# tonandr/keras_unsupervised

Hardware: AMD Instinct MI355X
Metric: cd1_gibbs_steps_per_sec (higher is better)
Workload: dtype f32 (storage, accumulation, results); products as exact bf16 triples on the bf16 MFMA (x3), the 0/1 x 0/1 product of the positive statistics on the fp8 MFMA (exact); 1 GPU; rbm_784x1024_cd1_batch4096_fp32 (BASELINE.json configs[1]); n_vis=784, n_hid=1024, batch_per_gpu=4096, global_batch=4096, cd_k=1, update_mode=fused, lr=1e-3/4096, parallelism=dp1, compute=x3

## Files before the change

keras_unsupervised_amd/csrc/kurbm_api.hip:

```cpp
#include <hip/hip_runtime.h>

#include <cstdarg>
#include <cstdio>
#include <cstdlib>
#include <cstring>
#include <string>

#include "../../include/kurbm.h"
#include "kurbm_kernels.h"
#include "kurbm_comm.h"

using namespace kurbm;

enum { KN_LDPAD, KN_X3_F8POS, KN_X3_BYTES, KN_X3_STATS_TALL, KN_BF16_SPLIT, KN_X3_FULL, KN_X3_TALL, KN_X3_MFAST, KN_X3_STATS_MFAST,
       KN_UNFUSED_MIRROR, KN_X3_XCD2D, KN_REDUCE_TR, KN_DP_CHUNKS, KN_X3_STATS_BYTES, KN_MAP_SLOW, KN_X3_PAIR, KN_X3_SPLIT_STATS, KN_X3_ATR, KN_SMALL_LOCAL,
       KN_COUNT };
constexpr int KN_AUTO = -1;
static const struct { const char* env; int dflt; } KNOBS[KN_COUNT] = {
    {"KURBM_LDPAD", 0},
    {"KURBM_X3_F8POS", 1},
    {"KURBM_X3_BYTES", 1},
    {"KURBM_X3_STATS_TALL", 1},
    {"KURBM_BF16_SPLIT", KN_AUTO},
    {"KURBM_X3_FULL", 0},
    {"KURBM_X3_TALL", KN_AUTO},
    {"KURBM_X3_MFAST", 1},
    {"KURBM_X3_STATS_MFAST", 0},
    {"KURBM_UNFUSED_MIRROR", 0},
    {"KURBM_X3_XCD2D", 1},
    {"KURBM_REDUCE_TR", 0},
    {"KURBM_DP_CHUNKS", 0},
    {"KURBM_X3_STATS_BYTES", 1},
    {"KURBM_MAP_SLOW", 0},
    {"KURBM_X3_PAIR", 1},
    {"KURBM_X3_SPLIT_STATS", 1},
    {"KURBM_X3_ATR", 1},
    {"KURBM_SMALL_LOCAL", 1},
};

constexpr size_t STATUS_BYTES = 4096;
struct kurbm_ctx {
    int device;
    int ncu;
    int force_cfg[3];
    int force_split;
    int tile_major;
    int knob[KN_COUNT];
    int xcc_round_robin;
    unsigned xcc_map;
    unsigned* status;
};

// ... 1114 lines not shown
    const size_t mb = carve_mirror(ctx, nullptr, p->n_vis, p->n_hid, pieces).bytes;
    if (mb > mirror_bytes) return fail(KURBM_ERR_WORKSPACE, "mirror too small: need %zu bytes, got %zu", mb, mirror_bytes);
    const size_t wb = carve_bf16(ctx, nullptr, rows > 0 ? rows : 1, p->n_vis, p->n_hid, pieces, v_pieces).bytes;
    if (wb > workspace_bytes) return fail(KURBM_ERR_WORKSPACE, "workspace too small: need %zu bytes, got %zu", wb, workspace_bytes);
    return KURBM_OK;
}

static bool split_stats_on(const kurbm_ctx* ctx, int pieces, int v_pieces) {
    return pieces == 3 && v_pieces == 3 && ctx->knob[KN_X3_SPLIT_STATS] != 0 && ctx->knob[KN_X3_BYTES] != 0;
}

static bool atr_on(const kurbm_ctx* ctx, int pieces, int v_pieces, bool gauss) {
    return gauss && split_stats_on(ctx, pieces, v_pieces) && ctx->knob[KN_X3_ATR] != 0 && ctx->knob[KN_X3_PAIR] != 0 && ctx->knob[KN_LDPAD] == 0;
}

static int cd_step_any(kurbm_ctx* ctx, int pieces, int v_pieces, const kurbm_params* p, void* mirror, size_t mirror_bytes,
                       const float* v_batch, int rows, int ldv, const kurbm_cd_opts* o, int which, void* workspace,
                       size_t workspace_bytes, kurbm_stream_t stream, int only = -1, int m_lo = 0, int m_hi = -1,
                       const kurbm_momentum* mom = nullptr) {
#define KURBM_STAGE(n) (only < 0 || only == (n) || (only == 8 && (n) <= 3) || (only == 7 && ((n) == 4 || (n) == 5)))
    if (m_hi < 0) m_hi = p ? p->n_vis : 0;
    if (int e = check_cd_args(ctx, pieces, v_pieces, p, mirror, mirror_bytes, v_batch, rows, ldv, o, workspace, workspace_bytes, false)) return e;
    if (mom) {
        if (int e = check_mom(mom, o)) return e;
        if (only >= 0) return fail(KURBM_ERR_ARG, "momentum applies to whole steps only");
    }
    const bool v_binary = (v_pieces == (1 | KURBM_V_BINARY));
    if (v_binary) v_pieces = 1;
    hipStream_t st = static_cast<hipStream_t>(stream);
    const Mirror m = carve_mirror(ctx, mirror, p->n_vis, p->n_hid, pieces);
    WorkspaceB w = carve_bf16(ctx, workspace, rows, p->n_vis, p->n_hid, pieces, v_pieces);

    const bool gauss = (o->mode == KURBM_MODE_VISIBLE_GAUSSIAN);
    const int act_h = gauss ? ACT_RELU : ACT_SIGMOID;
    const int act_v = gauss ? ACT_LINEAR : ACT_SIGMOID;
    const int noise_v = gauss ? NOISE_GAUSSIAN : NOISE_BERNOULLI;
    const uint32_t base = o->chain * 64u;
    const bool need_w = (which & 1) || o->delta_out;
    const int vn_pieces = (pieces == 3 && gauss) ? 3 : 1;
    const bool f8pos = v_binary && pieces == 3 && ctx->knob[KN_X3_F8POS] != 0;
    const bool byt = ctx->knob[KN_X3_BYTES] != 0;
    const bool hbytes = byt, vbytes = byt && v_binary && pieces == 3, nbytes = byt && !gauss;
    const bool tbytes = f8pos && nbytes && ctx->knob[KN_X3_STATS_BYTES] != 0 && ctx->knob[KN_X3_STATS_TALL] != 0 && p->n_vis > 128;
    const bool split_stats = split_stats_on(ctx, pieces, v_pieces);
    const bool tbytes_n = tbytes || (split_stats && nbytes);
    const bool vneg_tr = atr_on(ctx, pieces, v_pieces, gauss);
    int e;

    const int gp_v = ceil_div(rows, 64);
    const float* part_v_pos = nullptr;
    if (o->v_planes) {
        if (!aligned16(o->v_planes)) return fail(KURBM_ERR_ARG, "v_planes is misaligned");
        const VPlanes vp = carve_vplanes(ctx, o->v_planes, rows, p->n_vis, v_pieces);
        w.vb = vp.vb; w.vbT = vp.vbT; part_v_pos = vp.part_v;
    } else if (KURBM_STAGE(0))
        HIP_TRY(launch_f32_to_bf16(v_batch, rows, p->n_vis, ldv, w.vb, w.Lv, w.Kb, w.vbT, w.Lb, p->n_vis, v_pieces, w.planeV,
                                   w.planeVT, w.part_v, w.ldv32, st, f8pos ? 1 : 0, vbytes ? 1 : 0));
    RngArgs r = make_rng(o->seed, o->row0, base + 0u, o->step);
    if (KURBM_STAGE(1)) {
        HalfOutB ho;
        ho.out = w.hb; ho.ldo = w.Lh; ho.out_bytes = hbytes; ho.outT = w.hbT; ho.ldoT = w.Lb; ho.outT_f8 = f8pos; ho.outT_b8 = split_stats;
        ho.colpart = w.part_h; ho.ld_colpart = w.ldh32; ho.colsign = 1.f;
        if ((e = half_step_b(ctx, LAYOUT_VH, p, m, w.vb, w.Lv, v_pieces, w.planeV, rows, act_h, NOISE_BERNOULLI, &r, ho, st, vbytes))) return e;
    }
    const uint16_t* h_cur = w.hb;
    if (o->v_chain && KURBM_STAGE(1)) {
        HIP_TRY(launch_f32_to_bf16(o->v_chain, rows, p->n_vis, ldv, w.cb, w.Lv, w.Kb, nullptr, 0, 0, v_pieces, w.planeV, 0, nullptr, 0, st,
                                   0, vbytes ? 1 : 0));
        r = make_rng(o->seed, o->row0, base + 32u, o->step);
        HalfOutB ho;
        ho.out = w.h2b; ho.ldo = w.Lh; ho.out_bytes = hbytes;
        if ((e = half_step_b(ctx, LAYOUT_VH, p, m, w.cb, w.Lv, v_pieces, w.planeV, rows, act_h, NOISE_BERNOULLI, &r, ho, st, vbytes))) return e;
        h_cur = w.h2b;
    }
    int gm_v = ceil_div(rows, 128), gm_h = gm_v;
    for (int t = 1; t <= o->k; ++t) {
        const bool last = (t == o->k);
        r = make_rng(o->seed, o->row0, base + 2u * t - 1u, o->step);
        if (KURBM_STAGE(2)) {
            HalfOutB ho;
            ho.out = w.v2b; ho.ldo = w.Lv; ho.out_pieces = vn_pieces; ho.out_plane = w.planeV; ho.out_bytes = nbytes;
            if (last) {
                if (vneg_tr) ho.out_rows_pad = w.Kb;
                if (!vneg_tr) { ho.outT = w.v2bT; ho.ldoT = w.Lb; ho.outT_pieces = vn_pieces; ho.outT_plane = w.planeVT; ho.outT_b8 = tbytes_n; }
                ho.out_f32 = o->v_chain; ho.ldo32 = ldv;
                ho.grid_m_out = &gm_v;
            }
            ho.colpart = last ? w.part_v + (size_t)gp_v * w.ldv32 : nullptr; ho.ld_colpart = w.ldv32;
            ho.colsign = -1.f;
            if ((e = half_step_b(ctx, LAYOUT_HV, p, m, h_cur, w.Lh, 1, 0, rows, act_v, noise_v, &r, ho, st, hbytes))) return e;
        }
        if (!last && KURBM_STAGE(2)) {
            r = make_rng(o->seed, o->row0, base + 2u * t, o->step);
            HalfOutB ho;
            ho.out = w.h2b; ho.ldo = w.Lh; ho.out_bytes = hbytes;
            if ((e = half_step_b(ctx, LAYOUT_VH, p, m, w.v2b, w.Lv, vn_pieces, w.planeV, rows, act_h, NOISE_BERNOULLI, &r, ho, st, nbytes))) return e;
            h_cur = w.h2b;
        }
    }
// ... 87 lines not shown
            g.pb_max = 3;
            g.nseg = pb_codes(ctx, 1, 3, 0u, &g.seg_codes, 0);
            g.m_fastest = ctx->knob[KN_X3_STATS_MFAST];
            g.nkt = q.nkt; g.inv_nkt = inv_of(g.nkt);
            g.kt_total = q.kt_total; g.kt_per_split = q.kt_per_split; g.nsplit = q.nsplit;
            g.xcd2d = ctx->knob[KN_X3_XCD2D]; g.map_force = ctx->knob[KN_MAP_SLOW];
            HIP_TRY(launch_gemm_pb(EPI_SLAB, g, st));
        }
    } else if (need_w && KURBM_STAGE(4)) {
        GemmArgsB g;
        memset(&g, 0, sizeof g);
        g.A0 = w.vbT + (size_t)m_lo * w.Lb; g.a_plane0 = w.planeVT; g.B0 = w.hbT;
        g.A1 = w.v2bT + (size_t)m_lo * w.Lb; g.a_plane1 = w.planeVT; g.B1 = w.hnT; g.b_plane1 = w.planeHT;
        g.lda = w.Lb; g.ldb = w.Lb;
        if (tbytes) { g.a_bytes = 1; g.lda = 2 * w.Lb; }
        g.M = Mr; g.N = p->n_hid; g.K = w.Kb;
        g.grid_m = pl.gm; g.grid_n = pl.gn;
        g.slab = w.slab; g.slab_stride = slab_stride; g.ld_slab = pl.ld_slab;
        g.nseg = pb_codes(ctx, v_pieces, 1, 0u, &g.seg_codes, 0);
        g.nseg = pb_codes(ctx, vn_pieces, pieces, 1u, &g.seg_codes, g.nseg);
        g.pb_max = pieces;
        g.seg_fastest = 1; g.inv_nseg = inv_of(g.nseg);
        if (f8pos) { g.f8pos = 1; g.inv_nseg = inv_of(2 * g.nseg - 1); }
        g.m_fastest = ctx->knob[KN_X3_STATS_MFAST];
        g.cfg = pl.cfg;
        g.nkt = pl.nkt; g.inv_nkt = inv_of(g.nkt);
        g.kt_total = pl.kt_total; g.kt_per_split = pl.kt_per_split; g.nsplit = pl.nsplit;
        g.xcd2d = ctx->knob[KN_X3_XCD2D]; g.map_force = ctx->knob[KN_MAP_SLOW];
        HIP_TRY(launch_gemm_pb(EPI_SLAB, g, st));
    }
// ... 308 lines not shown
    a.rows = rows; a.n_vis = p->n_vis; a.ldv = ldv; a.ldv1 = w.ldv32; a.ncol_tiles = ncol0; a.ncol_tiles1 = ncol1; a.ld_rowpart = ld_rp;
    HIP_TRY(launch_score(a, st));
    return KURBM_OK;
}

int kurbm_x3_dump_plane(kurbm_ctx* ctx, int which, int rows, int n_vis, int n_hid, int v_pieces, int mode, const void* workspace,
                        size_t workspace_bytes, float* out, int ld_out, kurbm_stream_t stream) {
    if (!ctx || !workspace || !out) return fail(KURBM_ERR_ARG, "null argument");
    const bool v_binary = (v_pieces == (1 | KURBM_V_BINARY));
    if (v_binary) v_pieces = 1;
    if (rows <= 0 || n_vis <= 0 || n_hid <= 0 || (v_pieces != 1 && v_pieces != 3)) return fail(KURBM_ERR_ARG, "bad shape / v_pieces");
    const WorkspaceB w = carve_bf16(ctx, const_cast<void*>(workspace), rows, n_vis, n_hid, 3, v_pieces);
    if (w.bytes > workspace_bytes) return fail(KURBM_ERR_WORKSPACE, "workspace too small");
    const bool gauss = (mode == KURBM_MODE_VISIBLE_GAUSSIAN), byt = ctx->knob[KN_X3_BYTES] != 0;
    const bool f8pos = v_binary && ctx->knob[KN_X3_F8POS] != 0;
    DumpArgs a;
    memset(&a, 0, sizeof a);
    a.out = out; a.rows = rows; a.ld_out = ld_out; a.pieces = 1; a.sign = 1.f;
    switch (which) {
        case KURBM_PLANE_H_POS:   a.src = w.hb;   a.units = n_hid; a.ld = w.Lh; a.fmt = byt ? 1 : 0; break;
        case KURBM_PLANE_H_POS_T: a.src = w.hbT;  a.units = n_hid; a.ld = w.Lb; a.fmt = f8pos ? 2 : 0; a.transposed = 1;
                                  if (split_stats_on(ctx, 3, v_pieces)) { a.fmt = 1; a.ld = 2 * w.Lb; }
                                  break;
        case KURBM_PLANE_V_NEG:   a.src = w.v2b;  a.units = n_vis; a.ld = w.Lv; a.fmt = (byt && !gauss) ? 1 : 0;
                                  a.pieces = gauss ? 3 : 1; a.plane = w.planeV; break;
        case KURBM_PLANE_V_NEG_T: a.src = w.v2bT; a.units = n_vis; a.ld = w.Lb; a.transposed = 1;
                                  a.pieces = gauss ? 3 : 1; a.plane = w.planeVT;
                                  if (atr_on(ctx, 3, v_pieces, gauss)) {
                                      a.src = w.v2b; a.ld = w.Lv; a.transposed = 0; a.plane = w.planeV;
                                  }
                                  if ((f8pos && byt && !gauss && ctx->knob[KN_X3_STATS_BYTES] != 0 && ctx->knob[KN_X3_STATS_TALL] != 0 && n_vis > 128) ||
                                      (split_stats_on(ctx, 3, v_pieces) && !gauss)) {
                                      a.fmt = 1; a.ld = 2 * w.Lb;
                                  }
                                  break;
        case KURBM_PLANE_H_NEG_T: a.src = w.hnT;  a.units = n_hid; a.ld = w.Lb; a.transposed = 1; a.pieces = 3; a.plane = w.planeHT;
                                  a.sign = -1.f; break;
        default: return fail(KURBM_ERR_ARG, "unknown plane %d", which);
    }
    if (ld_out < a.units) return fail(KURBM_ERR_ARG, "ld_out < units");
    HIP_TRY(launch_dump_plane(a, static_cast<hipStream_t>(stream)));
    return KURBM_OK;
}

static int cd_epoch_x3_any(kurbm_ctx* ctx, const kurbm_params* p, void* mirror, size_t mirror_bytes, const float* V,
                           int v_pieces, int n_rows, int ldv, int batch_size, const kurbm_cd_opts* opts, void* workspace,
                           size_t workspace_bytes, kurbm_stream_t stream, const kurbm_momentum* mom) {
    if (!ctx || !opts) return fail(KURBM_ERR_ARG, "null argument");
    if (n_rows < 0 || batch_size <= 0) return fail(KURBM_ERR_ARG, "bad row count / batch size");
// ... 93 lines not shown
        if (b > bound[nc] && b < p->n_vis) bound[++nc] = b;
    }
    bound[++nc] = p->n_vis;
    kurbm_cd_opts o = *opts;
    o.apply = 0;
    const bool apply_ranges = opts->apply && nc > 1 && (p->n_hid & 3) == 0;
    if (rows == 0) HIP_TRY(hipMemsetAsync(o.delta_out, 0, ntot * sizeof(float), st));
    else if (nc > 1)
        if (int e = cd_step_any(ctx, pieces, v_pieces, p, mirror, mirror_bytes, v_batch, rows, ldv, &o, 7, workspace, workspace_bytes, stream, 8))
            return e;
    int err = KURBM_OK;
    bool on_comm = false;
    auto range = [&](int c) -> int {
        if (rows > 0) {
            const int e = (nc == 1)
                ? cd_step_any(ctx, pieces, v_pieces, p, mirror, mirror_bytes, v_batch, rows, ldv, &o, 7, workspace, workspace_bytes, stream)
                : cd_step_any(ctx, pieces, v_pieces, p, mirror, mirror_bytes, v_batch, rows, ldv, &o, 7, workspace, workspace_bytes, stream, 7,
                              bound[c], bound[c + 1]);
            if (e) return e;
        }
        const size_t lo = (size_t)bound[c] * p->n_hid, hi = (c + 1 == nc) ? ntot : (size_t)bound[c + 1] * p->n_hid;
        if (nc == 1)
            return comm_allreduce_sum(comm, o.delta_out + lo, hi - lo, st);
        HIP_TRY(hipEventRecord(comm->ev_ready[c], st));
        HIP_TRY(hipStreamWaitEvent(comm->stream, comm->ev_ready[c], 0));
        on_comm = true;
        if (int e = comm_allreduce_sum(comm, o.delta_out + lo, hi - lo, comm->stream)) return e;
        if (apply_ranges)
            return apply_delta_rows(ctx, p, mirror, mirror_bytes, pieces, o.delta_out, o.lr, 7, bound[c], bound[c + 1], c + 1 == nc, comm->stream);
        return KURBM_OK;
    };
// ... 18 lines not shown
int kurbm_cd_step_x3_peer(kurbm_ctx* ctx, kurbm_peer* peer, const kurbm_params* p, void* mirror, size_t mirror_bytes,
                          const float* v_batch, int v_pieces, int rows, int ldv, const kurbm_cd_opts* opts, void* workspace,
                          size_t workspace_bytes, kurbm_stream_t stream) {
    if (!ctx || !peer || !opts) return fail(KURBM_ERR_ARG, "null argument");
    if (int e = check_params(p)) return e;
    if (int e = peer_geometry_ok(peer, ctx->device, p->n_vis, p->n_hid)) return e;
    if (!opts->apply) return fail(KURBM_ERR_ARG, "kurbm_cd_step_x3_peer applies the summed update in place: apply = 1");
    if (rows < 0) return fail(KURBM_ERR_ARG, "rows must be >= 0");
    if (int e = check_cd_args(ctx, 3, v_pieces, p, mirror, mirror_bytes, v_batch, rows, ldv, opts, workspace, workspace_bytes, true)) return e;
    hipStream_t st = static_cast<hipStream_t>(stream);
    const size_t nw = (size_t)p->n_vis * p->n_hid, ntot = nw + p->n_hid + p->n_vis;
    kurbm_cd_opts o = *opts;
    o.apply = 0;
    o.delta_out = peer_delta(peer);
    if (rows == 0) HIP_TRY(hipMemsetAsync(o.delta_out, 0, ntot * sizeof(float), st));
    else if (int e = cd_step_any(ctx, 3, v_pieces, p, mirror, mirror_bytes, v_batch, rows, ldv, &o, 7, workspace, workspace_bytes, stream)) return e;
    PeerSrc src;
    if (int e = peer_exchange_shot1(peer, ctx->status, st, &src)) return e;
    const Mirror m = carve_mirror(ctx, mirror, p->n_vis, p->n_hid, 3);
    ReduceArgs a;
    memset(&a, 0, sizeof a);
    a.slab = src.own_sum; a.slab_stride = 0; a.nslab = 1; a.ld_slab = p->n_hid;
    a.n_vis = p->n_vis; a.n_hid = p->n_hid; a.ldw = p->ldw; a.lr = o.lr;
    a.W = p->W;
    a.part_h = src.own_sum + nw; a.nrow_tiles_h = 1; a.ld_part_h = p->n_hid; a.b_h = p->b_h;
    a.part_v = src.own_sum + nw + p->n_hid; a.nrow_tiles_v = 1; a.ld_part_v = p->n_vis; a.b_v = p->b_v;
    a.Wb = m.Wb; a.ldWb = m.ldW; a.planeWb = m.planeW;
    a.Wtb = m.Wtb; a.ldWtb = m.ldWt; a.planeWtb = m.planeWt; a.pieces = 3;
    a.tile_rows = ctx->knob[KN_REDUCE_TR];
    HIP_TRY(launch_reduce_apply_split(a, st, &src));
    return KURBM_OK;
// ... 77 lines not shown
```

keras_unsupervised_amd/csrc/kurbm_kernels.h:

```cpp
#pragma once
#include <hip/hip_runtime.h>
#include <stdint.h>

namespace kurbm {

enum { ACT_SIGMOID = 0, ACT_RELU = 1, ACT_LINEAR = 2 };
enum { NOISE_NONE = 0, NOISE_BERNOULLI = 1, NOISE_GAUSSIAN = 2 };
enum { EPI_HALFSTEP = 0, EPI_SLAB = 1, EPI_SOFTPLUS = 2, EPI_AIS = 3 };
enum { LAYOUT_VH = 0, LAYOUT_HV = 1, LAYOUT_OUTER = 2 };
enum { CFG_128x128 = 0, CFG_128x112 = 1, CFG_112x128 = 2, CFG_128x64 = 3, CFG_64x128 = 4, CFG_64x64 = 5,
       CFG_64x112 = 6, CFG_112x64 = 7, CFG_COUNT = 8 };

struct RngArgs {
    uint32_t seed_lo, seed_hi;
    uint32_t stream_id, step;
    uint64_t row0;
};

struct GemmArgs {
    const float* A0;
    const float* B0;
    const float* A1;
    const float* B1;
    int lda, ldb;
// ... 230 lines not shown
    int outT_f8;
    int outT_neg;
    size_t outT_plane;
    float* out_f32;
    float* prob_f32;
    float* out_u;
    int ldo32;
    float* colpart;
    int ld_colpart;
    float colsign;
    float* slab;
    size_t slab_stride;
    int ld_slab;
    int slab_t;
    int a_tr;
    int pair_ok;
    int map_force;
    int xcd2d;
    float* rowpart;
    int ld_rowpart;
    int rp;
    unsigned long long* stamps;
};

struct DumpArgs {
    const void* src;
    float* out;
    int rows, units, ld, ld_out, fmt, transposed, pieces;
    size_t plane;
    float sign;
// ... 52 lines not shown
```

keras_unsupervised_amd/csrc/kurbm_x3.hip:

```cpp
#include <hip/hip_runtime.h>
#include <hip/hip_ext.h>
#include <stdint.h>
#include <stdlib.h>

#include <type_traits>

#include "kurbm_kernels.h"
#include "kurbm_device.h"

namespace kurbm {

typedef __bf16 bf16x8 __attribute__((ext_vector_type(8)));
typedef uint32_t u32x4 __attribute__((ext_vector_type(4)));
typedef uint32_t u32x2 __attribute__((ext_vector_type(2)));

#ifdef KURBM_STAMPS
#define KURBM_STAMP(var)                                                                        \
    do {                                                                                        \
        __builtin_amdgcn_sched_barrier(0);                                                      \
        asm volatile("s_memtime %0\n\ts_waitcnt lgkmcnt(0)" : "=s"(var)::"memory");             \
        __builtin_amdgcn_sched_barrier(0);                                                      \
    } while (0)
#else
#define KURBM_STAMP(var) do { } while (0)
// ... 125 lines not shown
        const int tmn = bid - z * tiles_mn;
        const int q2 = div_map(tmn, g.m_fastest ? g.grid_m : g.grid_n, g.map_inv_b, g.map_slow);
        bm = g.m_fastest ? tmn - q2 * g.grid_m : q2;
        bn = g.m_fastest ? q2 : tmn - q2 * g.grid_n;
    }
    const int m0 = bm * BM, n0 = bn * BN;
    KURBM_PSTAMP(4);

    const int t_begin = z * g.kt_per_split;
    int t_end = t_begin + g.kt_per_split;
    if (t_end > g.kt_total) t_end = g.kt_total;
    const int nt = (t_end > t_begin && !(EPI == EPI_HALFSTEP && n0 >= g.N)) ? t_end - t_begin : 0;

    constexpr bool ATR = BSP && EPI == EPI_SLAB;
    const bool a_tr = ATR && g.a_tr != 0;
    unsigned goffA[NA], goffB[NB1];
#pragma unroll
    for (int it = 0; it < NA; ++it) {
        const int q = it * NTS + stid, row = q / CPR, ch = q % CPR;
        const int x = (m0 + row < g.M) ? m0 + row : 0;
        goffA[it] = AB ? (unsigned)(x * g.lda + 16 * (ch ^ ((row >> 1) & 7))) : 2u * (unsigned)(x * g.lda + 8 * (ch ^ ((row >> 1) & 7)));
        if (a_tr) {
            const int rt = q >> 4, ct = q & 15;
            goffA[it] = 2u * (unsigned)(rt * g.lda + m0 + 8 * (ct ^ (((rt & 3) << 2) | ((rt >> 2) & 3))));
        }
    }
#pragma unroll
    for (int it = 0; it < NB1; ++it) {
        const int q = it * NTS + stid, row = q / CPR, ch = q % CPR;
        const int x = (n0 + row < g.N) ? n0 + row : 0;
// ... 96 lines not shown
                    }
#endif
                    return;
                }
            }
            const unsigned char* c = smem + (bsp ? buf * A_BYTES : buf * STAGE) + (wm * WM + l15) * ROWB + 16 * ((4 * ks + slot) ^ swz);
#pragma unroll
            for (int mi = 0; mi < TM; ++mi) f[mi] = *reinterpret_cast<const u32x4*>(c + mi * 16 * ROWB);
        }
    };
    auto frag_b = [&](int buf, int ks, int p, u32x4 (&f)[TN]) __attribute__((always_inline)) {
        const unsigned char* c = smem + (bsp ? BSP_BOFF + buf * B_BYTES : buf * STAGE + B_OFF) + p * B1_BYTES + (wn * WN + l15) * ROWB +
                                 16 * ((4 * ks + slot) ^ swz);
#pragma unroll
        for (int ni = 0; ni < TN; ++ni) f[ni] = *reinterpret_cast<const u32x4*>(c + ni * 16 * ROWB);
    };
    [[maybe_unused]] u32x4 fx[AB ? TM : 1];
    auto expand_a = [&](int ks) __attribute__((always_inline)) {
        if constexpr (AB) {
#pragma unroll
            for (int mi = 0; mi < TM; ++mi) {
                const uint32_t lo = ks ? fa[0][mi].z : fa[0][mi].x, hi = ks ? fa[0][mi].w : fa[0][mi].y;
                fx[mi] = u32x4{__builtin_amdgcn_perm(0u, lo, 0x010C000Cu), __builtin_amdgcn_perm(0u, lo, 0x030C020Cu),
                               __builtin_amdgcn_perm(0u, hi, 0x010C000Cu), __builtin_amdgcn_perm(0u, hi, 0x030C020Cu)};
            }
        }
    };
    auto mfmas = [&](const afrag (&a)[TM], const u32x4 (&b)[TN]) __attribute__((always_inline)) {
#pragma unroll
        for (int mi = 0; mi < TM; ++mi) {
// ... 238 lines not shown
                }
                for (; i < nt; ++i) {
                    if (i + 3 < nt) __builtin_amdgcn_s_waitcnt(vm(NPT));
                    else __builtin_amdgcn_s_waitcnt(VM0);
                    __builtin_amdgcn_s_barrier();
                }
                KURBM_LSTAMP_OUT();
            } else if constexpr (ABS) {
                static_assert(NA / 2 + 3 * NB1 == 10 && NA + NB1 == 10, "10 pieces per wave and tile");
                const int nu = nt / 3;
                TileRef rp = tile_of(t_begin), rn = tile_of(t_begin + 1);
                TileRef ra = rn;
                ra.oa = rn.oa >> 1;
                int bf = 0, bb = 1;
                auto nxt = [](int b, int by) constexpr { return (b + by) % 3; };
                dma_part(2, rp, 3, bf);
                dma_part(0, ra, 1, bb);
                dma_part(0, rn, 2);
                __builtin_amdgcn_s_waitcnt(vm(NA + 3 * NB1));
                __builtin_amdgcn_s_setprio(KURBM_PRIO_LOADER);
                __builtin_amdgcn_s_barrier();
                rn.ob += 128u;
                for (int u = 0; u < nu; ++u) {
                    const bool more = u + 1 < nu;
                    const int bf1 = nxt(bf, 2), bb1 = nxt(bb, 2);
                    KURBM_LSTAMP(0);
                    if (more) { rp.oa += 128u; rp.ob += 128u; dma_part(0, rp, 1, bf1, 0, NA / 2); }
                    dma_part(1, rn, 2);
                    rn.ob += 128u;
                    KURBM_LSTAMP(1);
                    if (more) __builtin_amdgcn_s_waitcnt(vm(10)); else __builtin_amdgcn_s_waitcnt(vm(3 * NB1));
                    KURBM_LSTAMP(2);
                    __builtin_amdgcn_s_barrier();
                    KURBM_LSTAMP(3);
                    if (more) {
                        ra.oa += 128u;
                        dma_part(0, ra, 1, bb1, 0, NA / 2);
                        dma_part(2, rp, 2);
                        dma_part(0, rp, 1, bf1, NA / 2, NA);
                        __builtin_amdgcn_s_waitcnt(vm(10));
                    } else {
                        __builtin_amdgcn_s_waitcnt(VM0);
                    }
                    __builtin_amdgcn_s_barrier();
                    if (more) {
                        dma_part(0, rn, 2);
                        rn.ob += 128u;
                        dma_part(0, ra, 1, bb1, NA / 2, NA);
                        __builtin_amdgcn_s_waitcnt(vm(10));
                    } else {
                        __builtin_amdgcn_s_waitcnt(VM0);
                    }
                    __builtin_amdgcn_s_barrier();
                    bf = bf1; bb = bb1;
                }
                KURBM_LSTAMP_OUT();
            } else if constexpr (AB) {
                TileRef ra = tile_of(t_begin);
                TileRef rb = ra;
                const uint32_t ob0 = ra.ob;
                ra.neg = false; ra.oa = 128u * (uint32_t)(t_begin >> 1);
                KURBM_PSTAMP(0);
                dma_part(0, ra, 3, 0);
// ... 146 lines not shown
            for (int ni = 0; ni < NI_LDS; ++ni)
#pragma unroll
                for (int mi = 0; mi < TM; ++mi) {
                    const uint64_t grow = g.rng.row0 + (uint64_t)(m0 + wm * WM + slot * 4 + mi * 16);
                    uint32_t w[4];
                    philox4x32_10((uint32_t)(n0 + wn * WN + l15 + ni * 16), (uint32_t)(grow >> 2), g.rng.stream_id, g.rng.step,
                                  g.rng.seed_lo, g.rng.seed_hi, w);
                    *reinterpret_cast<u32x4*>(smem + SMEM_BYTES + ((ni * TM + mi) * NT + tid) * 16) = u32x4{w[0], w[1], w[2], w[3]};
                }
        }
    }
    __builtin_amdgcn_s_setprio(KURBM_PRIO_MFMA);
    if (nt > 0) {
        __syncthreads();
        frag_a(0, 0, fa[0]);
        frag_b(ABS ? 2 : 0, 0, 0, fb[0]);
        if constexpr (!ABS) expand_a(0);
        KURBM_STAMP(ts[1]);
        int i = 0;
        if constexpr (ABS) {
            const uint32_t arow = (uint32_t)((wm * WM + l15) * ROWB);
            uint32_t of8 = 0u, oby = A_BYTES;
            auto rd_f8 = [&](uint32_t off, int ks, afrag (&f)[TM]) __attribute__((always_inline)) {
                const unsigned char* c = smem + (arow + 16 * ((4 * ks + slot) ^ swz) + off);
#pragma unroll
                for (int mi = 0; mi < TM; ++mi) f[mi] = *reinterpret_cast<const u32x4*>(c + mi * 16 * ROWB);
            };
            auto rd_by = [&](uint32_t off, int half, afrag (&f)[TM]) __attribute__((always_inline)) {
                const unsigned char* c = smem + (arow + 16 * ((4 * half + slot) ^ swz) + off);
#pragma unroll
                for (int mi = 0; mi < TM; ++mi) f[mi] = *reinterpret_cast<const u32x4*>(c + mi * 16 * ROWB);
// ... 5 lines not shown
#pragma unroll
                for (int mi = 0; mi < TM; ++mi) {
                    const uint32_t lo = ks ? fa[0][mi].z : fa[0][mi].x, hi = ks ? fa[0][mi].w : fa[0][mi].y;
                    fa[1][mi] = u32x4{__builtin_amdgcn_perm(0u, lo, 0x010C000Cu), __builtin_amdgcn_perm(0u, lo, 0x030C020Cu),
                                      __builtin_amdgcn_perm(0u, hi, 0x010C000Cu), __builtin_amdgcn_perm(0u, hi, 0x030C020Cu)};
                }
            };
            auto mf = [&](const u32x4 (&b)[TN]) __attribute__((always_inline)) {
#pragma unroll
                for (int mi = 0; mi < TM; ++mi)
#pragma unroll
                    for (int ni = 0; ni < TN; ++ni)
                        acc[mi][ni] = __builtin_amdgcn_mfma_f32_16x16x32_bf16(
                            __builtin_bit_cast(bf16x8, fa[1][mi]), __builtin_bit_cast(bf16x8, b[ni]), acc[mi][ni], 0, 0, 0);
            };
            auto f8t = [&]() __attribute__((always_inline)) {
                typedef int i32x8 __attribute__((ext_vector_type(8)));
                __builtin_amdgcn_sched_barrier(0);
                rd_f8(of8, 1, fa[1]);
                frag_b(2, 1, 0, fb[1]);
#pragma unroll
                for (int mi = 0; mi < TM; ++mi)
#pragma unroll
                    for (int ni = 0; ni < TN; ++ni) {
                        const i32x8 a = {(int)fa[0][mi].x, (int)fa[0][mi].y, (int)fa[0][mi].z, (int)fa[0][mi].w,
                                         (int)fa[1][mi].x, (int)fa[1][mi].y, (int)fa[1][mi].z, (int)fa[1][mi].w};
                        const i32x8 b = {(int)fb[0][ni].x, (int)fb[0][ni].y, (int)fb[0][ni].z, (int)fb[0][ni].w,
                                         (int)fb[1][ni].x, (int)fb[1][ni].y, (int)fb[1][ni].z, (int)fb[1][ni].w};
                        acc[mi][ni] = __builtin_amdgcn_mfma_scale_f32_16x16x128_f8f6f4(a, b, acc[mi][ni], 0, 0, 0, 0x80, 0, 0x7F);
                    }
                __builtin_amdgcn_sched_barrier(0);
                __syncthreads();
                __builtin_amdgcn_sched_barrier(0);
                rd_by(oby, 0, fa[0]);
                frag_b(0, 0, 0, fb[0]);
                __builtin_amdgcn_sched_barrier(0);
                expand0(0);
                __builtin_amdgcn_sched_barrier(0);
            };
            auto negt = [&](const int half, const uint32_t nf8) __attribute__((always_inline)) {
#pragma unroll
                for (int u = 0; u < 6; ++u) {
                    __builtin_amdgcn_sched_barrier(0);
                    if (u == 0) { frag_b(half, 0, 1, fb[1]); frag_b(half, 0, 2, fb[2]); }
                    if (u == 1) frag_b(half, 1, 0, fb[0]);
                    if (u == 2) frag_b(half, 1, 1, fb[1]);
                    if (u == 3) frag_b(half, 1, 2, fb[2]);
                    if (u == 5) {
                        __syncthreads();
                        __builtin_amdgcn_sched_barrier(0);
                        if (half == 0) { rd_by(oby, 1, fa[0]); frag_b(1, 0, 0, fb[0]); }
                        else { rd_f8(nf8, 0, fa[0]); frag_b(2, 0, 0, fb[0]); }
                    }
                    mf(fb[u % 3]);
                    if (u == 2) { __builtin_amdgcn_sched_barrier(0); expand0(1); }
                    if (u == 5 && half == 0) { __builtin_amdgcn_sched_barrier(0); expand0(0); }
                }
                __builtin_amdgcn_sched_barrier(0);
            };
            for (; i + 2 < nt; i += 3) {
                const uint32_t nf8 = adv(of8);
                f8t();
                negt(0, nf8);
                negt(1, nf8);
                of8 = nf8; oby = adv(oby);
            }
        } else if constexpr (DEEP) {
            const uint32_t la = (uint32_t)((wm * WM + l15) * ROWB + 16 * (slot ^ swz));
            const uint32_t lb = (uint32_t)(B_OFF + (wn * WN + l15) * ROWB + 16 * (slot ^ swz));
            auto rd_a = [&](uint32_t blk_off, int half, afrag (&f)[TM]) __attribute__((always_inline)) {
                const unsigned char* c = smem + ((la ^ (64u * (uint32_t)half)) + blk_off);
#pragma unroll
                for (int mi = 0; mi < TM; ++mi) f[mi] = *reinterpret_cast<const u32x4*>(c + mi * 16 * ROWB);
            };
            auto rd_b = [&](uint32_t stg_off, int ks, u32x4 (&f)[TN]) __attribute__((always_inline)) {
                const unsigned char* c = smem + ((lb ^ (64u * (uint32_t)ks)) + stg_off);
#pragma unroll
                for (int ni = 0; ni < TN; ++ni) f[ni] = *reinterpret_cast<const u32x4*>(c + ni * 16 * ROWB);
            };
            auto expand_from = [&](const afrag (&f)[TM], int ks) __attribute__((always_inline)) {
#pragma unroll
// ... 439 lines not shown
            for (int mi = 0; mi < TM; ++mi)
#pragma unroll
                for (int r = 0; r < 4; ++r)
                    smem[(wm * WM + mi * 16 + slot * 4 + r) * PROWB + kperm64(wn * WN + ni * 16 + l15)] =
                        (col_ok && xv[mi][ni][r] != 0.f) ? (unsigned char)0x40 : (unsigned char)0;
        }
        __syncthreads();
        constexpr int CHB = BN / 16;
        unsigned char* plane = reinterpret_cast<unsigned char*>(g.out);
#pragma unroll
        for (int q8 = 0; q8 < (BM * CHB + NT - 1) / NT; ++q8) {
            const int q = q8 * NT + tid, row = q / CHB, c = q % CHB;
            const int gr = m0 + row, gc = n0 + 16 * c;
            if (row < BM && gr < g.M && gc < g.ldo_cols)
                *reinterpret_cast<u32x4*>(plane + (size_t)gr * g.ldo + gc) = *reinterpret_cast<const u32x4*>(smem + row * PROWB + 16 * c);
        }
    } else if (g.out) {
        const int odd = l15 & 1;
        const uint32_t sel = odd ? 0x03020706u : 0x05040100u;
        const int npc = (g.out_pieces == 3) ? 3 : 1;
#pragma unroll
        for (int ni = 0; ni < TN; ++ni)
            if (!(colb + ni * 16 < g.N)) {
#pragma unroll
                for (int mi = 0; mi < TM; ++mi)
#pragma unroll
                    for (int r = 0; r < 4; ++r) xv[mi][ni][r] = 0.f;
            }
        for (int j = 0; j < npc; ++j) {
            if (j > 0) __syncthreads();
// ... 123 lines not shown
                    const long long cost = (long long)(g.nsplit / xz) * ((long long)(g.grid_m / xr) * bmr * wa + (long long)(g.grid_n / xc) * bnr * wb);
                    if (best < 0 || cost < best) { best = cost; g.xcd_r = xr; g.xcd_c = xc; }
                }
        }
    }
    {
        const bool tri = g.pb_max == 3 && !g.a_bytes && g.nseg == 3 && g.seg_fastest && ((g.seg_codes >> 4) & 1ull) == ((g.seg_codes >> 9) & 1ull) &&
                         ((g.seg_codes >> 4) & 1ull) == ((g.seg_codes >> 14) & 1ull) &&
                         (g.seg_codes & 0x7FFFull & ~0x4210ull) == ((0ull | (3ull << 2)) | ((1ull | (2ull << 2)) << 5) | ((2ull | (1ull << 2)) << 10));
        g.bshare = (tri && g.pair_ok && g.cfg == 0 && (epi == EPI_HALFSTEP ? (g.nsplit == 1 && !((g.seg_codes >> 4) & 1ull)) : (epi == EPI_SLAB && !g.f8pos)) &&
                    g.kt_per_split % 3 == 0 && g.kt_total % 3 == 0) ? 2 : 0;
    }
    if (g.a_tr && !(g.bshare == 2 && epi == EPI_SLAB)) return hipErrorInvalidValue;
    g.walk3 = (epi == EPI_SLAB && g.pb_max == 3 && g.f8pos && g.nseg == 2 && ((g.seg_codes >> 7) & 3u) == 3u &&
               g.kt_per_split % 3 == 0 && g.kt_total % 3 == 0) ? 1 : 0;
    {
        if (nblk <= 0) return hipErrorInvalidValue;
        {
            const unsigned long long lim = 0xFFFFFFFFull;
            unsigned long long worst;
            if (g.xcd_r) {
                const unsigned long long rl = (unsigned long long)(g.grid_m / g.xcd_r), cl = (unsigned long long)(g.grid_n / g.xcd_c);
                worst = (unsigned long long)(nblk / 8 + 1) * (rl * cl);
                const unsigned long long w2 = (rl * cl) * (rl > cl ? rl : cl);
                if (w2 > worst) worst = w2;
            } else {
                const unsigned long long tm = (unsigned long long)g.grid_m * (unsigned long long)g.grid_n;
                worst = (unsigned long long)nblk * tm;
                const unsigned long long w2 = tm * (unsigned long long)(g.grid_m > g.grid_n ? g.grid_m : g.grid_n);
                if (w2 > worst) worst = w2;
// ... 36 lines not shown
```

Before: 10280 steps/s (1 step = CD-1 update over 4096 rows, 784x1024 fp32).

## Read row-major byte planes via LDS transpose loads instead of writing transposed copies

Adds a default-on tr8 path for the binary-visible x3 statistics GEMM. The half-steps no longer write transposed h_pos and v_neg byte/fp8 planes. Instead they pad the row-major byte outputs with zero rows, and the stats kernel DMAs the row-major planes into LDS and uses ds_read_tr8_b64 to build the MFMA fragments. This removes the transposed-output stores and their bandwidth from the sampling epilogues. In exchange it adds swizzled address math, a changed scale constant for the fp8 MFMA, and extra validity checks, with the data-parallel and chunked paths excluded.

```diff
diff --git a/keras_unsupervised_amd/csrc/kurbm_api.hip b/keras_unsupervised_amd/csrc/kurbm_api.hip
--- a/keras_unsupervised_amd/csrc/kurbm_api.hip
+++ b/keras_unsupervised_amd/csrc/kurbm_api.hip
@@ -13,7 +13,7 @@
 using namespace kurbm;
 
 enum { KN_LDPAD, KN_X3_F8POS, KN_X3_BYTES, KN_X3_STATS_TALL, KN_BF16_SPLIT, KN_X3_FULL, KN_X3_TALL, KN_X3_MFAST, KN_X3_STATS_MFAST,
-       KN_UNFUSED_MIRROR, KN_X3_XCD2D, KN_REDUCE_TR, KN_DP_CHUNKS, KN_X3_STATS_BYTES, KN_MAP_SLOW, KN_X3_PAIR, KN_X3_SPLIT_STATS, KN_X3_ATR, KN_SMALL_LOCAL,
+       KN_UNFUSED_MIRROR, KN_X3_XCD2D, KN_REDUCE_TR, KN_DP_CHUNKS, KN_X3_STATS_BYTES, KN_MAP_SLOW, KN_X3_PAIR, KN_X3_SPLIT_STATS, KN_X3_ATR, KN_SMALL_LOCAL, KN_X3_STATS_TR8,
        KN_COUNT };
 constexpr int KN_AUTO = -1;
 static const struct { const char* env; int dflt; } KNOBS[KN_COUNT] = {
@@ -36,6 +36,7 @@
     {"KURBM_X3_SPLIT_STATS", 1},
     {"KURBM_X3_ATR", 1},
     {"KURBM_SMALL_LOCAL", 1},
+    {"KURBM_X3_STATS_TR8", 1},
 };
 
 constexpr size_t STATUS_BYTES = 4096;
@@ -1180,10 +1181,14 @@
     return gauss && split_stats_on(ctx, pieces, v_pieces) && ctx->knob[KN_X3_ATR] != 0 && ctx->knob[KN_X3_PAIR] != 0 && ctx->knob[KN_LDPAD] == 0;
 }
 
+static bool stats_tr8_on(const kurbm_ctx* ctx, bool tbytes) {
+    return tbytes && ctx->knob[KN_X3_STATS_TR8] != 0 && ctx->knob[KN_LDPAD] == 0;
+}
+
 static int cd_step_any(kurbm_ctx* ctx, int pieces, int v_pieces, const kurbm_params* p, void* mirror, size_t mirror_bytes,
                        const float* v_batch, int rows, int ldv, const kurbm_cd_opts* o, int which, void* workspace,
                        size_t workspace_bytes, kurbm_stream_t stream, int only = -1, int m_lo = 0, int m_hi = -1,
-                       const kurbm_momentum* mom = nullptr) {
+                       const kurbm_momentum* mom = nullptr, bool dp = false) {
 #define KURBM_STAGE(n) (only < 0 || only == (n) || (only == 8 && (n) <= 3) || (only == 7 && ((n) == 4 || (n) == 5)))
     if (m_hi < 0) m_hi = p ? p->n_vis : 0;
     if (int e = check_cd_args(ctx, pieces, v_pieces, p, mirror, mirror_bytes, v_batch, rows, ldv, o, workspace, workspace_bytes, false)) return e;
@@ -1210,6 +1215,8 @@
     const bool tbytes = f8pos && nbytes && ctx->knob[KN_X3_STATS_BYTES] != 0 && ctx->knob[KN_X3_STATS_TALL] != 0 && p->n_vis > 128;
     const bool split_stats = split_stats_on(ctx, pieces, v_pieces);
     const bool tbytes_n = tbytes || (split_stats && nbytes);
+    const bool stats_tr8 = stats_tr8_on(ctx, tbytes) && !dp && only != 7 && only != 8 && m_lo == 0 && m_hi == p->n_vis;
+    const int rows_pad8 = stats_tr8_on(ctx, tbytes) ? w.Kb : 0;
     const bool vneg_tr = atr_on(ctx, pieces, v_pieces, gauss);
     int e;
 
@@ -1225,7 +1232,9 @@
     RngArgs r = make_rng(o->seed, o->row0, base + 0u, o->step);
     if (KURBM_STAGE(1)) {
         HalfOutB ho;
-        ho.out = w.hb; ho.ldo = w.Lh; ho.out_bytes = hbytes; ho.outT = w.hbT; ho.ldoT = w.Lb; ho.outT_f8 = f8pos; ho.outT_b8 = split_stats;
+        ho.out = w.hb; ho.ldo = w.Lh; ho.out_bytes = hbytes;
+        ho.out_rows_pad = rows_pad8;
+        if (!stats_tr8) { ho.outT = w.hbT; ho.ldoT = w.Lb; ho.outT_f8 = f8pos; ho.outT_b8 = split_stats; }
         ho.colpart = w.part_h; ho.ld_colpart = w.ldh32; ho.colsign = 1.f;
         if ((e = half_step_b(ctx, LAYOUT_VH, p, m, w.vb, w.Lv, v_pieces, w.planeV, rows, act_h, NOISE_BERNOULLI, &r, ho, st, vbytes))) return e;
     }
@@ -1247,8 +1256,8 @@
             HalfOutB ho;
             ho.out = w.v2b; ho.ldo = w.Lv; ho.out_pieces = vn_pieces; ho.out_plane = w.planeV; ho.out_bytes = nbytes;
             if (last) {
-                if (vneg_tr) ho.out_rows_pad = w.Kb;
-                if (!vneg_tr) { ho.outT = w.v2bT; ho.ldoT = w.Lb; ho.outT_pieces = vn_pieces; ho.outT_plane = w.planeVT; ho.outT_b8 = tbytes_n; }
+                ho.out_rows_pad = vneg_tr ? w.Kb : rows_pad8;
+                if (!vneg_tr && !stats_tr8) { ho.outT = w.v2bT; ho.ldoT = w.Lb; ho.outT_pieces = vn_pieces; ho.outT_plane = w.planeVT; ho.outT_b8 = tbytes_n; }
                 ho.out_f32 = o->v_chain; ho.ldo32 = ldv;
                 ho.grid_m_out = &gm_v;
             }
@@ -1366,6 +1375,11 @@
         g.A1 = w.v2bT + (size_t)m_lo * w.Lb; g.a_plane1 = w.planeVT; g.B1 = w.hnT; g.b_plane1 = w.planeHT;
         g.lda = w.Lb; g.ldb = w.Lb;
         if (tbytes) { g.a_bytes = 1; g.lda = 2 * w.Lb; }
+        if (stats_tr8) {
+            g.tr8 = 1;
+            g.B0 = w.hb; g.ldb_tr = w.Lh;
+            g.A1 = w.v2b; g.lda_tr = w.Lv;
+        }
         g.M = Mr; g.N = p->n_hid; g.K = w.Kb;
         g.grid_m = pl.gm; g.grid_n = pl.gn;
         g.slab = w.slab; g.slab_stride = slab_stride; g.ld_slab = pl.ld_slab;
@@ -1704,6 +1718,7 @@
     if (w.bytes > workspace_bytes) return fail(KURBM_ERR_WORKSPACE, "workspace too small");
     const bool gauss = (mode == KURBM_MODE_VISIBLE_GAUSSIAN), byt = ctx->knob[KN_X3_BYTES] != 0;
     const bool f8pos = v_binary && ctx->knob[KN_X3_F8POS] != 0;
+    const bool tbytes = f8pos && byt && !gauss && ctx->knob[KN_X3_STATS_BYTES] != 0 && ctx->knob[KN_X3_STATS_TALL] != 0 && n_vis > 128;
     DumpArgs a;
     memset(&a, 0, sizeof a);
     a.out = out; a.rows = rows; a.ld_out = ld_out; a.pieces = 1; a.sign = 1.f;
@@ -1711,6 +1726,9 @@
         case KURBM_PLANE_H_POS:   a.src = w.hb;   a.units = n_hid; a.ld = w.Lh; a.fmt = byt ? 1 : 0; break;
         case KURBM_PLANE_H_POS_T: a.src = w.hbT;  a.units = n_hid; a.ld = w.Lb; a.fmt = f8pos ? 2 : 0; a.transposed = 1;
                                   if (split_stats_on(ctx, 3, v_pieces)) { a.fmt = 1; a.ld = 2 * w.Lb; }
+                                  if (stats_tr8_on(ctx, tbytes)) {
+                                      a.src = w.hb; a.ld = w.Lh; a.fmt = 1; a.transposed = 0;
+                                  }
                                   break;
         case KURBM_PLANE_V_NEG:   a.src = w.v2b;  a.units = n_vis; a.ld = w.Lv; a.fmt = (byt && !gauss) ? 1 : 0;
                                   a.pieces = gauss ? 3 : 1; a.plane = w.planeV; break;
@@ -1719,10 +1737,10 @@
                                   if (atr_on(ctx, 3, v_pieces, gauss)) {
                                       a.src = w.v2b; a.ld = w.Lv; a.transposed = 0; a.plane = w.planeV;
                                   }
-                                  if ((f8pos && byt && !gauss && ctx->knob[KN_X3_STATS_BYTES] != 0 && ctx->knob[KN_X3_STATS_TALL] != 0 && n_vis > 128) ||
-                                      (split_stats_on(ctx, 3, v_pieces) && !gauss)) {
+                                  if (tbytes || (split_stats_on(ctx, 3, v_pieces) && !gauss)) {
                                       a.fmt = 1; a.ld = 2 * w.Lb;
                                   }
+                                  if (stats_tr8_on(ctx, tbytes)) { a.src = w.v2b; a.ld = w.Lv; a.fmt = 1; a.transposed = 0; a.plane = w.planeV; }
                                   break;
         case KURBM_PLANE_H_NEG_T: a.src = w.hnT;  a.units = n_hid; a.ld = w.Lb; a.transposed = 1; a.pieces = 3; a.plane = w.planeHT;
                                   a.sign = -1.f; break;
@@ -1846,7 +1864,8 @@
     auto range = [&](int c) -> int {
         if (rows > 0) {
             const int e = (nc == 1)
-                ? cd_step_any(ctx, pieces, v_pieces, p, mirror, mirror_bytes, v_batch, rows, ldv, &o, 7, workspace, workspace_bytes, stream)
+                ? cd_step_any(ctx, pieces, v_pieces, p, mirror, mirror_bytes, v_batch, rows, ldv, &o, 7, workspace, workspace_bytes, stream, -1, 0, -1,
+                              nullptr, true)
                 : cd_step_any(ctx, pieces, v_pieces, p, mirror, mirror_bytes, v_batch, rows, ldv, &o, 7, workspace, workspace_bytes, stream, 7,
                               bound[c], bound[c + 1]);
             if (e) return e;
@@ -1895,7 +1914,8 @@
     o.apply = 0;
     o.delta_out = peer_delta(peer);
     if (rows == 0) HIP_TRY(hipMemsetAsync(o.delta_out, 0, ntot * sizeof(float), st));
-    else if (int e = cd_step_any(ctx, 3, v_pieces, p, mirror, mirror_bytes, v_batch, rows, ldv, &o, 7, workspace, workspace_bytes, stream)) return e;
+    else if (int e = cd_step_any(ctx, 3, v_pieces, p, mirror, mirror_bytes, v_batch, rows, ldv, &o, 7, workspace, workspace_bytes, stream, -1, 0, -1,
+                                 nullptr, true)) return e;
     PeerSrc src;
     if (int e = peer_exchange_shot1(peer, ctx->status, st, &src)) return e;
     const Mirror m = carve_mirror(ctx, mirror, p->n_vis, p->n_hid, 3);
diff --git a/keras_unsupervised_amd/csrc/kurbm_kernels.h b/keras_unsupervised_amd/csrc/kurbm_kernels.h
--- a/keras_unsupervised_amd/csrc/kurbm_kernels.h
+++ b/keras_unsupervised_amd/csrc/kurbm_kernels.h
@@ -268,6 +268,8 @@
     int ld_slab;
     int slab_t;
     int a_tr;
+    int tr8;
+    int lda_tr, ldb_tr;
     int pair_ok;
     int map_force;
     int xcd2d;
diff --git a/keras_unsupervised_amd/csrc/kurbm_x3.hip b/keras_unsupervised_amd/csrc/kurbm_x3.hip
--- a/keras_unsupervised_amd/csrc/kurbm_x3.hip
+++ b/keras_unsupervised_amd/csrc/kurbm_x3.hip
@@ -163,6 +163,7 @@
 
     constexpr bool ATR = BSP && EPI == EPI_SLAB;
     const bool a_tr = ATR && g.a_tr != 0;
+    const bool tr8 = ABS && g.tr8 != 0;
     unsigned goffA[NA], goffB[NB1];
 #pragma unroll
     for (int it = 0; it < NA; ++it) {
@@ -289,6 +290,41 @@
                                  16 * ((4 * ks + slot) ^ swz);
 #pragma unroll
         for (int ni = 0; ni < TN; ++ni) f[ni] = *reinterpret_cast<const u32x4*>(c + ni * 16 * ROWB);
+    };
+    [[maybe_unused]] uint32_t a8[2] = {0u, 0u}, b8[2] = {0u, 0u};
+    if (tr8) {
+        const int q8 = l15 >> 1, p8 = l15 & 1;
+#pragma unroll
+        for (int e = 0; e < 2; ++e) {
+            a8[e] = (uint32_t)(256 * (8 * slot + q8) + 16 * ((4 * wm + 2 * e + p8) ^ (2 * q8)));
+            b8[e] = (uint32_t)(2 * STAGE + B_OFF + 64 * (16 * slot + q8) + 16 * ((2 * e + p8) ^ (2 * ((q8 >> 2) & 1))) + 8 * wn);
+        }
+    }
+    auto tr8_rd = [&](uint32_t off) __attribute__((always_inline)) {
+        u32x2 r = u32x2{0u, 0u};
+#if defined(__HIP_DEVICE_COMPILE__)
+        typedef int v2i __attribute__((ext_vector_type(2)));
+        typedef __attribute__((address_space(3))) v2i* lds_v2i;
+        const v2i t = __builtin_amdgcn_ds_read_tr8_b64_v2i32((lds_v2i)(smem + off));
+        r = u32x2{(uint32_t)t.x, (uint32_t)t.y};
+#endif
+        return r;
+    };
+    auto rd_f8b_tr = [&](int ks, u32x4 (&f)[TN]) __attribute__((always_inline)) {
+        static_assert(!ABS || TN == 2, "tr8: two 16-column blocks per wave");
+#pragma unroll
+        for (int ni = 0; ni < TN; ++ni) {
+            const u32x2 lo = tr8_rd(b8[ni & 1] + 4096 * ks), hi = tr8_rd(b8[ni & 1] + 4096 * ks + 512);
+            f[ni] = u32x4{lo.x, lo.y, hi.x, hi.y};
+        }
+    };
+    auto rd_by_tr = [&](uint32_t off, int half, afrag (&f)[TM]) __attribute__((always_inline)) {
+#pragma unroll
+        for (int mi = 0; mi < TM; ++mi) {
+            const uint32_t o = off + a8[mi & 1] + 8 * (mi >> 1) + 256 * 64 * half;
+            const u32x2 k0 = tr8_rd(o), k1 = tr8_rd(o + 256 * 32);
+            f[mi] = u32x4{k0.x, k0.y, k1.x, k1.y};
+        }
     };
     [[maybe_unused]] u32x4 fx[AB ? TM : 1];
     auto expand_a = [&](int ks) __attribute__((always_inline)) {
@@ -557,8 +593,53 @@
                 ra.oa = rn.oa >> 1;
                 int bf = 0, bb = 1;
                 auto nxt = [](int b, int by) constexpr { return (b + by) % 3; };
-                dma_part(2, rp, 3, bf);
-                dma_part(0, ra, 1, bb);
+                [[maybe_unused]] unsigned gA8[NA], gB8[NB1];
+                if (tr8) {
+                    const int lw = wave - NT / 64;
+#pragma unroll
+                    for (int it = 0; it < NA; ++it) {
+                        const int row = 4 * (it * 4 + lw) + (lane >> 4);
+                        int col = m0 + 16 * ((lane & 15) ^ (2 * (row & 7)));
+                        if (col >= g.lda_tr) col = m0;
+                        gA8[it] = (unsigned)(row * g.lda_tr + col);
+                    }
+#pragma unroll
+                    for (int it = 0; it < NB1; ++it) {
+                        const int row = 16 * (it * 4 + lw) + (lane >> 2);
+                        gB8[it] = (unsigned)(row * g.ldb_tr + n0 + 16 * ((lane & 3) ^ (2 * ((row >> 2) & 1))));
+                    }
+                }
+                auto dma_by = [&](int blk, int a_lo, int a_hi) __attribute__((always_inline)) {
+                    if (tr8) {
+#if defined(__HIP_DEVICE_COMPILE__)
+                        typedef __attribute__((address_space(3))) void* lds_ptr;
+                        unsigned char* a = smem + blk * A_BYTES + (wave - NT / 64) * 8 * ROWB;
+                        const uint32_t so = ra.oa * (uint32_t)g.lda_tr;
+#pragma unroll
+                        for (int it = 0; it < NA; ++it)
+                            if (it >= a_lo && it < a_hi)
+                                __builtin_amdgcn_raw_ptr_buffer_load_lds(dA1, (lds_ptr)(a + it * 32 * ROWB), 16, gA8[it], so, 0, 0);
+#endif
+                    } else {
+                        dma_part(0, ra, 1, blk, a_lo, a_hi);
+                    }
+                };
+                auto dma_f8b = [&]() __attribute__((always_inline)) {
+                    if (tr8) {
+#if defined(__HIP_DEVICE_COMPILE__)
+                        typedef __attribute__((address_space(3))) void* lds_ptr;
+                        unsigned char* b = smem + 2 * STAGE + B_OFF + (wave - NT / 64) * 8 * ROWB;
+                        const uint32_t so = g.offB0 + (rp.ob - g.offB0) * (uint32_t)g.ldb_tr;
+#pragma unroll
+                        for (int it = 0; it < NB1; ++it)
+                            __builtin_amdgcn_raw_ptr_buffer_load_lds(dB, (lds_ptr)(b + it * 32 * ROWB), 16, gB8[it], so, 0, 0);
+#endif
+                    } else {
+                        dma_part(2, rp, 2);
+                    }
+                };
+                dma_part(2, rp, 1, bf); dma_f8b();
+                dma_by(bb, 0, NA);
                 dma_part(0, rn, 2);
                 __builtin_amdgcn_s_waitcnt(vm(NA + 3 * NB1));
                 __builtin_amdgcn_s_setprio(KURBM_PRIO_LOADER);
@@ -578,8 +659,8 @@
                     KURBM_LSTAMP(3);
                     if (more) {
                         ra.oa += 128u;
-                        dma_part(0, ra, 1, bb1, 0, NA / 2);
-                        dma_part(2, rp, 2);
+                        dma_by(bb1, 0, NA / 2);
+                        dma_f8b();
                         dma_part(0, rp, 1, bf1, NA / 2, NA);
                         __builtin_amdgcn_s_waitcnt(vm(10));
                     } else {
@@ -589,7 +670,7 @@
                     if (more) {
                         dma_part(0, rn, 2);
                         rn.ob += 128u;
-                        dma_part(0, ra, 1, bb1, NA / 2, NA);
+                        dma_by(bb1, NA / 2, NA);
                         __builtin_amdgcn_s_waitcnt(vm(10));
                     } else {
                         __builtin_amdgcn_s_waitcnt(VM0);
@@ -766,7 +847,8 @@
     if (nt > 0) {
         __syncthreads();
         frag_a(0, 0, fa[0]);
-        frag_b(ABS ? 2 : 0, 0, 0, fb[0]);
+        if (tr8) rd_f8b_tr(0, fb[0]);
+        else frag_b(ABS ? 2 : 0, 0, 0, fb[0]);
         if constexpr (!ABS) expand_a(0);
         KURBM_STAMP(ts[1]);
         int i = 0;
@@ -802,11 +884,15 @@
                         acc[mi][ni] = __builtin_amdgcn_mfma_f32_16x16x32_bf16(
                             __builtin_bit_cast(bf16x8, fa[1][mi]), __builtin_bit_cast(bf16x8, b[ni]), acc[mi][ni], 0, 0, 0);
             };
+            auto units = [&](auto tr_tag) __attribute__((always_inline)) {
+            constexpr bool TR = decltype(tr_tag)::value;
+            constexpr int sca = TR ? 0x7F : 0x80;
             auto f8t = [&]() __attribute__((always_inline)) {
                 typedef int i32x8 __attribute__((ext_vector_type(8)));
                 __builtin_amdgcn_sched_barrier(0);
                 rd_f8(of8, 1, fa[1]);
-                frag_b(2, 1, 0, fb[1]);
+                if constexpr (TR) rd_f8b_tr(1, fb[1]);
+                else frag_b(2, 1, 0, fb[1]);
 #pragma unroll
                 for (int mi = 0; mi < TM; ++mi)
 #pragma unroll
@@ -815,12 +901,13 @@
                                          (int)fa[1][mi].x, (int)fa[1][mi].y, (int)fa[1][mi].z, (int)fa[1][mi].w};
                         const i32x8 b = {(int)fb[0][ni].x, (int)fb[0][ni].y, (int)fb[0][ni].z, (int)fb[0][ni].w,
                                          (int)fb[1][ni].x, (int)fb[1][ni].y, (int)fb[1][ni].z, (int)fb[1][ni].w};
-                        acc[mi][ni] = __builtin_amdgcn_mfma_scale_f32_16x16x128_f8f6f4(a, b, acc[mi][ni], 0, 0, 0, 0x80, 0, 0x7F);
+                        acc[mi][ni] = __builtin_amdgcn_mfma_scale_f32_16x16x128_f8f6f4(a, b, acc[mi][ni], 0, 0, 0, sca, 0, 0x7F);
                     }
                 __builtin_amdgcn_sched_barrier(0);
                 __syncthreads();
                 __builtin_amdgcn_sched_barrier(0);
-                rd_by(oby, 0, fa[0]);
+                if constexpr (TR) rd_by_tr(oby, 0, fa[0]);
+                else rd_by(oby, 0, fa[0]);
                 frag_b(0, 0, 0, fb[0]);
                 __builtin_amdgcn_sched_barrier(0);
                 expand0(0);
@@ -837,8 +924,15 @@
                     if (u == 5) {
                         __syncthreads();
                         __builtin_amdgcn_sched_barrier(0);
-                        if (half == 0) { rd_by(oby, 1, fa[0]); frag_b(1, 0, 0, fb[0]); }
-                        else { rd_f8(nf8, 0, fa[0]); frag_b(2, 0, 0, fb[0]); }
+                        if (half == 0) {
+                            if constexpr (TR) rd_by_tr(oby, 1, fa[0]);
+                            else rd_by(oby, 1, fa[0]);
+                            frag_b(1, 0, 0, fb[0]);
+                        } else {
+                            rd_f8(nf8, 0, fa[0]);
+                            if constexpr (TR) rd_f8b_tr(0, fb[0]);
+                            else frag_b(2, 0, 0, fb[0]);
+                        }
                     }
                     mf(fb[u % 3]);
                     if (u == 2) { __builtin_amdgcn_sched_barrier(0); expand0(1); }
@@ -853,6 +947,9 @@
                 negt(1, nf8);
                 of8 = nf8; oby = adv(oby);
             }
+            };
+            if (tr8) units(std::true_type{});
+            else units(std::false_type{});
         } else if constexpr (DEEP) {
             const uint32_t la = (uint32_t)((wm * WM + l15) * ROWB + 16 * (slot ^ swz));
             const uint32_t lb = (uint32_t)(B_OFF + (wn * WN + l15) * ROWB + 16 * (slot ^ swz));
@@ -1322,6 +1419,8 @@
             const int gr = m0 + row, gc = n0 + 16 * c;
             if (row < BM && gr < g.M && gc < g.ldo_cols)
                 *reinterpret_cast<u32x4*>(plane + (size_t)gr * g.ldo + gc) = *reinterpret_cast<const u32x4*>(smem + row * PROWB + 16 * c);
+            else if (row < BM && gr < g.out_rows_pad && gc < g.ldo_cols)
+                *reinterpret_cast<u32x4*>(plane + (size_t)gr * g.ldo + gc) = u32x4{0u, 0u, 0u, 0u};
         }
     } else if (g.out) {
         const int odd = l15 & 1;
@@ -1475,6 +1574,9 @@
     if (g.a_tr && !(g.bshare == 2 && epi == EPI_SLAB)) return hipErrorInvalidValue;
     g.walk3 = (epi == EPI_SLAB && g.pb_max == 3 && g.f8pos && g.nseg == 2 && ((g.seg_codes >> 7) & 3u) == 3u &&
                g.kt_per_split % 3 == 0 && g.kt_total % 3 == 0) ? 1 : 0;
+    if (g.tr8 && !(g.walk3 && g.a_bytes && g.cfg == 2 && g.lda_tr > 0 && g.ldb_tr > 0 && g.lda_tr % 16 == 0 && g.ldb_tr % 16 == 0 &&
+                   (unsigned long long)g.K * (unsigned long long)(g.lda_tr > g.ldb_tr ? g.lda_tr : g.ldb_tr) + g.offB0 < 0x7FFFFFFFull))
+        return hipErrorInvalidValue;
     {
         if (nblk <= 0) return hipErrorInvalidValue;
         {
```

Result: no change. 10250 steps/s (1 step = CD-1 update over 4096 rows, 784x1024 fp32) (-0.3%).
